# facebookresearch/unbiased-teacher-v2

Hardware: AMD Instinct MI355X
Metric: images/sec/node (labeled+unlabeled) UTv2 step, R50-FPN 1333x800 (higher is better)
Workload: dtype f16

## Files before the change

include/utv2.h:

```cpp
#ifndef UTV2_H
#define UTV2_H
#include <stdint.h>
#ifdef __cplusplus
extern "C" {
#endif

typedef struct ihipStream_t* utv2_stream_t;

int utv2_conv2d_nhwc_fwd(const float* x, const float* w, float* y, const float* scale, const float* bias,
                         const float* residual, int N, int H, int W, int C, int K, int KH, int KW, int stride, int pad,
                         int in_dil, int OH, int OW, int relu, int accumulate, int Kred, utv2_stream_t stream);
int utv2_conv2d_stem_fwd(const float* x, const float* w, void* y, int y_dtype, const float* scale, const float* bias, int N,
                         int H, int W, int K, int KH, int KW, int stride, int pad, int OH, int OW, int relu, int Kred,
                         utv2_stream_t stream);
int utv2_conv2d_wgrad_splits(int N, int OH, int OW, int K, int Kred);
int64_t utv2_conv2d_wgrad_workspace_floats(int N, int OH, int OW, int K, int Kred);
int utv2_conv2d_nhwc_wgrad(const float* x, const float* dy, float* dw, float* ws, int N, int H, int W, int C, int K,
                           int KH, int KW, int stride, int pad, int OH, int OW, int accumulate, utv2_stream_t stream);
int utv2_colsum(const float* g, float* db, float* ws, int M, int C, int accumulate, utv2_stream_t stream);
int utv2_weight_flip_transpose(const float* w, float* wt, int K, int KH, int KW, int C, utv2_stream_t stream);

int utv2_conv2d_ml_fwd(const float* x, const float* w, float* y, const float* scale, const float* bias,
                       const float* residual, int nlev, const int* H_host, const int* W_host, int N, int C, int K, int KH,
                       int KW, int pad, int relu, int accumulate, utv2_stream_t stream);
// ... 230 lines not shown
int utv2_roi_sample(const float* boxes, const unsigned char* valid, const float* max_iou, const int* argmax, const float* keys, int N, int P,
                    const float* gt_boxes, const int* gt_classes, const unsigned char* gt_valid, const float* gt_scores, const float* gt_std,
                    int G, float iou_thr, int num_classes, int batch, int nfg_max, float* out_boxes, int64_t* out_classes,
                    float* out_gt_boxes, unsigned char* out_valid, int64_t* out_idx, float* out_conf, float* out_std, utv2_stream_t stream);
int utv2_roi_box_loss(const float* deltas, const float* stdl, int64_t ld, const int64_t* cls, const float* prop, const float* gtb,
                      const float* gstd, int R, int num_classes, int nbox, int mode, float wx, float wy, float scale_clamp, float ts_better,
                      float t_cert, float* sum, float* gdeltas, float* gstd_out, utv2_stream_t stream);
int utv2_softmax_focal_fwd(const float* logits, const int* target, int R, int C, float gamma, float* loss_sum, float* ws,
                           utv2_stream_t stream);
int utv2_softmax_focal_bwd(const float* logits, const int* target, int R, int C, float gamma, const float* coef,
                           float* dlogits, utv2_stream_t stream);
int utv2_rcnn_loss_combine(const float* rpn_sup, const float* rpn_uns, const float* focal_sup, const float* focal_uns, const float* box_sup,
                           const float* box_uns, const int* tgt_sup, int n_sup, const int* tgt_uns, int n_uns, float rpn_norm_sup,
                           float rpn_norm_uns, float w_rpn_cls, float w_rpn_loc, float w_box, const float* wt_host, float* rec, float* coef,
                           utv2_stream_t stream);

int utv2_stem_pool_fwd_bf16(const void* xpad16, const void* w16s, void* y, const float* scale, const float* shift, int N, int H, int W,
                            int K, utv2_stream_t stream);

int utv2_bottleneck_supported(int C, int MID, int has_shortcut);
int utv2_bottleneck_fwd_bf16(const void* x, void* y, const void* w1, const void* w2, const void* w3, const void* wsc, const float* s1,
                             const float* b1, const float* s2, const float* b2, const float* s3, const float* b3, const float* ssc,
                             const float* bsc, int N, int H, int W, int C, int MID, utv2_stream_t stream);

int64_t utv2_aug_resize_workspace_bytes(int H, int W, int OH, int OW);
int utv2_aug_resize_bilinear_u8(const unsigned char* src, int H, int W, unsigned char* dst, int OH, int OW, int flip, void* ws,
                                utv2_stream_t stream);
int utv2_aug_gray_mean_u8(const unsigned char* img, int64_t npix, void* sum_ws, int* mean_out, utv2_stream_t stream);
int utv2_aug_blend_u8(unsigned char* img, int64_t npix, int mode, float alpha, const int* mean, utv2_stream_t stream);
int utv2_aug_hue_u8(unsigned char* img, int64_t npix, int shift, utv2_stream_t stream);
int utv2_aug_grayscale_u8(unsigned char* img, int64_t npix, utv2_stream_t stream);
int utv2_aug_box_blur_u8(const unsigned char* src, unsigned char* dst, int H, int W, int vertical, int radius, int ww, int fw,
                         utv2_stream_t stream);
int utv2_aug_erase_u8(unsigned char* img, int H, int W, int i, int j, int h, int w, const float* noise, utv2_stream_t stream);
int utv2_aug_hwc_to_chw_u8(const unsigned char* src, unsigned char* dst, int64_t npix, utv2_stream_t stream);

int utv2_coco_pair_keys(const float* scores, const int* cls, const long long* off, int N, int K, long long* keys, utv2_stream_t stream);
int utv2_coco_seg_offsets(const long long* keys, int64_t n, int64_t nseg, long long* off, utv2_stream_t stream);
int utv2_coco_rank_keys(const long long* key1, const long long* pair_off, int64_t D, int K, int max_dets, long long* key2,
                        unsigned char* rank, utv2_stream_t stream);
int64_t utv2_coco_eval_workspace_bytes(int64_t D, int K);
int utv2_coco_match(const float* dbox, const long long* dperm, const long long* dpair_off, const double* gbox, const unsigned char* gcrowd,
                    const double* garea, const long long* gperm, const long long* gpair_off, int N, int K, int64_t D, int max_dets,
                    int max_gt, const double* iou_thrs_host, const double* area_rng_host, void* ws, utv2_stream_t stream);
int utv2_coco_accumulate(const long long* perm2, const long long* cat_off, const unsigned char* rank, int K, int64_t D,
                         const double* rec_thrs_host, const void* ws, double* precision, double* recall, utv2_stream_t stream);
// ... 16 lines not shown
```

unbiased-teacher-v2_amd/csrc/bottleneck.hip:

```cpp
#include "common.h"

#define BT_TH 8
#define BT_TW 16
#define BT_HW 18
#define BT_HALO 180
#define BT_HP 192
#define BT_COUT 256
#define BT_MID 64
#define BT_STAGE 16384
#define BT_C1 (BT_HP * 128)
#define BT_PRM 1280
#define BT_LDS (BT_STAGE + BT_C1 + BT_PRM * 4)

struct BtArgs {
  const h16_t* x;
  h16_t* y;
  const h16_t *w1, *w2, *w3, *wsc;
  const float *s1, *b1, *s2, *b2, *s3, *b3, *ssc, *bsc;
  int N, H, W, tiles_x, tiles_y, ntiles;
};

__device__ __forceinline__ bf16x8_t lds_frag(const unsigned char* smem, int off) { return *(const bf16x8_t*)(smem + off); }

template <int CIN, bool SC>
__global__ __launch_bounds__(256, 3) void bottleneck_fused(BtArgs a) {
  constexpr int NCH = CIN / 32;
  extern __shared__ __attribute__((aligned(16))) unsigned char smem[];
  unsigned char* stageA = smem;
  unsigned char* c1 = smem + BT_STAGE;
  unsigned char* stageB = smem + BT_STAGE;
  unsigned char* c2 = smem;
  unsigned char* w3l = smem + BT_STAGE;
  float* prm = (float*)(smem + BT_STAGE + BT_C1);
  const int tid = threadIdx.x, lane = tid & 63, wave = tid >> 6, l31 = lane & 31, fh = lane >> 5;

  int t;
  {
    const int bid = blockIdx.x, q = a.ntiles >> 3, r = a.ntiles & 7, xcd = bid & 7, idx = bid >> 3;
    t = (xcd < r ? xcd * (q + 1) : r * (q + 1) + (xcd - r) * q) + idx;
  }
  const int per = a.tiles_x * a.tiles_y;
  const int n = t / per, rem = t - n * per, ty = rem / a.tiles_x, tx = rem - ty * a.tiles_x;
  const int y0 = ty * BT_TH, x0 = tx * BT_TW;
  const h16_t* ximg = a.x + (size_t)n * a.H * a.W * CIN;

  const h16_t* xsrc[3];
  int xdst[3];
#pragma unroll
// ... 73 lines not shown
      *(bf16x8_t*)(nxt + wdst) = wr[(kc + 1) % 3];
    }
    __syncthreads();
  }

  {
    const int pbs[3] = {pbA, pbA, pbB}, cbs[3] = {0, 1, cbB};
#pragma unroll
    for (int i = 0; i < 3; ++i) {
      const int px = pbs[i] * 32 + l31;
      const int hy = px / BT_HW, hx = px - hy * BT_HW, gy = y0 - 1 + hy, gx = x0 - 1 + hx;
      const bool ok = px < BT_HALO && gy >= 0 && gy < a.H && gx >= 0 && gx < a.W;
#pragma unroll
      for (int q = 0; q < 4; ++q) {
        const int ch = cbs[i] * 32 + 8 * q + 4 * fh;
        const f32x4 sc = *(const f32x4*)(prm + ch), bi = *(const f32x4*)(prm + 64 + ch);
        bf16x4_t o;
#pragma unroll
        for (int j = 0; j < 4; ++j) {
          float v = acc1[i][4 * q + j] * sc[j] + bi[j];
          v = ok ? fmaxf(v, 0.f) : 0.f;
          o[j] = (h16_t)v;
        }
        *(bf16x4_t*)(c1 + px * 128 + (((cbs[i] * 4 + q) ^ (px & 7)) << 4) + fh * 8) = o;
      }
    }
  }
#pragma unroll
  for (int i = 0; i < 2; ++i) *(bf16x8_t*)(stageA + t2co[i] * 128 + ((t2slot ^ (t2co[i] & 7)) << 4)) = tr[0][i];
  __syncthreads();

  f32x16 acc2[2];
#pragma unroll
  for (int i = 0; i < 2; ++i)
#pragma unroll
    for (int e = 0; e < 16; ++e) acc2[i][e] = 0.f;
  const int p = wave * 32 + l31, pr = p >> 4, pc = p & 15;
  const int qco[2] = {tid >> 3, (tid + 256) >> 3}, qslot = tid & 7;
  bf16x8_t wq[2], sq[2];
#pragma unroll
  for (int tap = 0; tap < 9; ++tap) {
    unsigned char* cur = stageA + (tap & 1) * 8192;
    unsigned char* nxt = stageA + ((tap + 1) & 1) * 8192;
    if (tap + 3 < 9) {
#pragma unroll
      for (int i = 0; i < 2; ++i) tr[tap % 3][i] = *(const bf16x8_t*)(a.w2 + t2co[i] * 576 + (tap + 3) * 64 + t2slot * 8);
    } else if (tap == 6) {
#pragma unroll
      for (int i = 0; i < 2; ++i) {
        wq[i] = *(const bf16x8_t*)(a.w3 + qco[i] * BT_MID + qslot * 8);
        if constexpr (SC) sq[i] = *(const bf16x8_t*)(a.wsc + qco[i] * CIN + qslot * 8);
      }
    }
    const int dy = tap / 3, dx = tap - dy * 3;
    const int h = (pr + dy) * BT_HW + pc + dx;
#pragma unroll
    for (int ks = 0; ks < 4; ++ks) {
      const int slot = ks * 2 + fh;
      const bf16x8_t xf = lds_frag(c1, h * 128 + ((slot ^ (h & 7)) << 4));
      const bf16x8_t wa = lds_frag(cur, w0row * 128 + ((slot ^ (w0row & 7)) << 4));
      const bf16x8_t wb = lds_frag(cur, w1row * 128 + ((slot ^ (w1row & 7)) << 4));
      acc2[0] = mfma_32x32x16(wa, xf, acc2[0]);
      acc2[1] = mfma_32x32x16(wb, xf, acc2[1]);
    }
    if (tap + 1 < 9) {
#pragma unroll
      for (int i = 0; i < 2; ++i) *(bf16x8_t*)(nxt + t2co[i] * 128 + ((t2slot ^ (t2co[i] & 7)) << 4)) = tr[(tap + 1) % 3][i];
    }
    __syncthreads();
  }
  const int sub = lane >> 3, cv = lane & 7;
  int opix[4];
#pragma unroll
  for (int i = 0; i < 4; ++i) {
    const int pp = wave * 32 + 8 * i + sub, gy = y0 + (pp >> 4), gx = x0 + (pp & 15);
    opix[i] = (gy < a.H && gx < a.W) ? ((gy * a.W + gx) * BT_COUT + cv * 8) : -1;
  }
  h16_t* yout = a.y + (size_t)n * a.H * a.W * BT_COUT;
  bf16x8_t res[2][4];
  bf16x8_t xf3[4];
  if constexpr (!SC) {
#pragma unroll
    for (int i = 0; i < 4; ++i) res[0][i] = opix[i] >= 0 ? *(const bf16x8_t*)(ximg + opix[i]) : zero8;
  } else {
    const int gy = y0 + pr, gx = x0 + pc;
    const bool in = gy < a.H && gx < a.W;
#pragma unroll
    for (int ks = 0; ks < 4; ++ks)
      xf3[ks] = in ? *(const bf16x8_t*)(ximg + ((size_t)gy * a.W + gx) * CIN + ks * 16 + fh * 8) : zero8;
  }
#pragma unroll
  for (int cb = 0; cb < 2; ++cb)
#pragma unroll
    for (int q = 0; q < 4; ++q) {
// ... 133 lines not shown
}

extern "C" {

int utv2_bottleneck_fwd_bf16(const void* x, void* y, const void* w1, const void* w2, const void* w3, const void* wsc, const float* s1,
                             const float* b1, const float* s2, const float* b2, const float* s3, const float* b3, const float* ssc,
                             const float* bsc, int N, int H, int W, int C, int MID, hipStream_t stream) {
  if (!x || !y || x == y || !w1 || !w2 || !w3 || !s1 || !b1 || !s2 || !b2 || !s3 || !b3 || N < 1 || H < 1 || W < 1) return UTV2_EARG;
  if (MID != BT_MID || !((C == 256 && !wsc) || (C == 64 && wsc && ssc && bsc))) return UTV2_EARG;
  if ((long long)H * W * BT_COUT > 0x7fffffffll) return UTV2_EARG;
  BtArgs a;
  a.x = (const h16_t*)x; a.y = (h16_t*)y; a.w1 = (const h16_t*)w1; a.w2 = (const h16_t*)w2; a.w3 = (const h16_t*)w3; a.wsc = (const h16_t*)wsc;
  a.s1 = s1; a.b1 = b1; a.s2 = s2; a.b2 = b2; a.s3 = s3; a.b3 = b3; a.ssc = ssc; a.bsc = bsc;
  a.N = N; a.H = H; a.W = W;
  a.tiles_x = cdiv(W, BT_TW); a.tiles_y = cdiv(H, BT_TH);
  const long long nt = (long long)N * a.tiles_x * a.tiles_y;
  if (nt > 0x7fffffff) return UTV2_EARG;
  a.ntiles = (int)nt;
  if (wsc) hipLaunchKernelGGL((bottleneck_fused<64, true>), dim3((unsigned)a.ntiles), dim3(256), BT_LDS, stream, a);
  else hipLaunchKernelGGL((bottleneck_fused<256, false>), dim3((unsigned)a.ntiles), dim3(256), BT_LDS, stream, a);
  return utv2_launch_status();
}

int utv2_bottleneck_supported(int C, int MID, int has_shortcut) {
  return MID == BT_MID && ((C == 256 && !has_shortcut) || (C == 64 && has_shortcut));
}

}
```

unbiased-teacher-v2_amd/ubteacher/hip.py:

```python
import ctypes
import os

import torch

_HERE = os.path.dirname(os.path.abspath(__file__))
_LIB_DIR = os.environ.get("UTV2_LIB_DIR") or os.path.join(os.path.dirname(_HERE), "lib")
LIB_PATH = os.path.join(_LIB_DIR, "libutv2_hip.so")
LIB_PATHS = {"bf16": LIB_PATH, "fp16": os.path.join(_LIB_DIR, "libutv2_hip_f16.so")}
H16 = ["bf16"]


_H16_DT = [torch.bfloat16]


def set_h16(kind):
    assert kind in LIB_PATHS
    H16[0] = kind
    _H16_DT[0] = torch.bfloat16 if kind == "bf16" else torch.float16


def h16_dtype():
    return _H16_DT[0]

_lib = None
# ... 989 lines not shown
        ri = rowinfo_nhwc(N, H, W, OH, OW, stride, pad, kh, kw, x.device)
    if relu_bits is not None:
        assert out.dtype == h16_dtype()
        relu_bits = _bits_ok(relu_bits, out.shape)
    call("utv2_conv2d_nhwc_fwd_bf16_bits", _p(x), _dt(x), _p(w16), _p(out), _same_dt(out, residual, mask, post_mask), _p(scale), _p(bias),
         _p(residual), _p(mask), _p(post_mask), N, H, W, C, K, kh, kw, stride, pad, in_dil, OH, OW, int(relu), int(accumulate), _p(ri),
         _p(relu_bits), None, None, _stream())
    return out


def bottleneck_fwd_bf16(x, w1, w2, w3, s1, b1, s2, b2, s3, b3, wsc=None, ssc=None, bsc=None, out=None):
    N, H, W, C = x.shape
    MID, K = w1.shape[0], w3.shape[0]
    assert x.dtype == h16_dtype() and w1.dtype == w2.dtype == w3.dtype == h16_dtype() and K == 256
    assert tuple(w1.shape) == (MID, C) and tuple(w2.shape) == (MID, 9 * MID) and tuple(w3.shape) == (K, MID)
    assert wsc is None or (tuple(wsc.shape) == (K, C) and wsc.dtype == h16_dtype())
    if out is None:
        out = torch.empty((N, H, W, K), dtype=x.dtype, device=x.device)
    call("utv2_bottleneck_fwd_bf16", _p(x), _p(out), _p(w1), _p(w2), _p(w3), _p(wsc), _p(s1), _p(b1), _p(s2), _p(b2), _p(s3), _p(b3),
         _p(ssc), _p(bsc), N, H, W, C, MID, _stream())
    return out


def bottleneck_supported(C, MID, has_shortcut):
    return bool(load().utv2_bottleneck_supported(C, MID, int(has_shortcut)))


def conv2d_dgrad_bf16(dy, wt16, in_shape, stride, pad, kh, kw, out=None, out_dtype=None, mask=None, residual=None, post_mask=None,
                      mask_bits=None, post_mask_bits=None):
    N, H, W, C = in_shape
    _, OH, OW, K = dy.shape
    if out is None:
        out = torch.empty((N, H, W, C), dtype=_act_dtype(dy, out_dtype), device=dy.device)
    ri = None
    if _CONV_ROWINFO and kh * kw > 1 and stride == 1 and dy.dtype == h16_dtype() and K % 32 == 0 and kh * kw <= 16 and OW < 32768:
        ri = rowinfo_nhwc(N, OH, OW, H, W, 1, kh - 1 - pad, kh, kw, dy.device)
    if mask_bits is not None or post_mask_bits is not None:
        assert out.dtype == h16_dtype() and (mask is None or mask_bits is None) and (post_mask is None or post_mask_bits is None)
        mask_bits = _bits_ok(mask_bits, out.shape) if mask_bits is not None else None
        post_mask_bits = _bits_ok(post_mask_bits, out.shape) if post_mask_bits is not None else None
    call("utv2_conv2d_nhwc_fwd_bf16_bits", _p(dy), _dt(dy), _p(wt16), _p(out), _same_dt(out, residual, mask, post_mask), None, None,
         _p(residual), _p(mask), _p(post_mask), N, OH, OW, K, C, kh, kw, 1, kh - 1 - pad, stride, H, W, 0, 0, _p(ri), None,
         _p(mask_bits), _p(post_mask_bits), _stream())
    return out


# ... 398 lines not shown
```

unbiased-teacher-v2_amd/ubteacher/modeling/backbone.py:

```python
import math
import os

import torch

from .. import hip, ops
from ..d2.registry import BACKBONE_REGISTRY


def _nchw_view(cout, cin, k):
    def fn(t):
        return t.view(cout, k, k, cin).permute(0, 3, 1, 2)
    return fn


def _msra_init(cout, cin, k):
    def fn(t):
        std = math.sqrt(2.0 / (cout * k * k))
        t.normal_(0.0, std)
    return fn


def _xavier_init(cout, cin, k):
    def fn(t):
        bound = math.sqrt(3.0 / (cin * k * k))
# ... 101 lines not shown
                 stride_in_1x1=True):
        self.out_features = out_features
        def stem_init(t):
            t.zero_()
            w = torch.empty(64, 7, 7, 3, device=t.device).normal_(0.0, math.sqrt(2.0 / (64 * 49)))
            t.view(64, 208)[:, :196].view(64, 7, 7, 4)[..., :3].copy_(w)
        stem_train = freeze_at < 1
        self.stem_w = store.new((64, 208), "decay" if stem_train else "frozen", stem_init).export(
            prefix + ".stem.conv1.weight", lambda t: torch.as_strided(t, (64, 3, 7, 7), (208, 1, 28, 4), t.storage_offset()))
        self.stem_bn = folder.add(FrozenBN(store, prefix + ".stem.conv1.norm", 64))
        self.stem = ops.Conv(self.stem_w, 4, 64, 7, 2, 3, bn=self.stem_bn, relu=True, trainable=stem_train, kred=208)
        self.stages = []
        cin = 64
        for si, nblocks in enumerate(num_blocks):
            name, mid, cout = "res%d" % (si + 2), groups * width_per_group * 2 ** si, 256 * 2 ** si
            trainable = freeze_at < si + 2
            blocks = []
            for b in range(nblocks):
                stride = 2 if (b == 0 and name != "res2") else 1
                blocks.append(Bottleneck(store, folder, "%s.%s.%d" % (prefix, name, b), cin, cout, mid, stride, trainable, groups,
                                         stride_in_1x1))
                cin = cout
            self.stages.append((name, blocks, trainable))
        self.channels = {"res2": 256, "res3": 512, "res4": 1024, "res5": 2048}
        self.strides = {"res2": 4, "res3": 8, "res4": 16, "res5": 32}

    def __call__(self, x4):
        outs = {}
        if self.stem.trainable and torch.is_grad_enabled():
            assert x4.dtype == torch.float32 and x4.shape[-1] == 4, "a trainable stem takes the fp32 NHWC4 image"
            x = ops.stem(self.stem, x4)
            for name, blocks, trainable in self.stages:
                for b in blocks:
                    x = b(x)
                if name in self.out_features:
                    outs[name] = x
            return outs
        sc, sh = self.stem.scale_shift()
        if x4.dtype == hip.h16_dtype():
            v = (self.stem_w.store.version, hip.H16[0])
            if getattr(self, "_w16s_version", None) != v:
                self._w16s = hip.stem_weight_image(self.stem_w.t)
                self._w16s_version = v
            if os.environ.get("UTV2_FUSED_STEM_POOL", "1") != "0" and self._w16s.shape[0] == 64:
                x = hip.stem_pool_fwd_bf16(x4, self._w16s, sc, sh)
            else:
                x = hip.maxpool3x3s2(hip.conv2d_stem_fwd_bf16(x4, self._w16s, sc, sh, True, hip.h16_dtype()))
        else:
            x = hip.maxpool3x3s2(hip.conv2d_stem_fwd(x4, self.stem_w.t, sc, sh, 2, 3, 7, 7, True, ops.act_dtype()))
        for name, blocks, trainable in self.stages:
            if trainable:
                for b in blocks:
                    x = b(x)
            else:
                with torch.no_grad():
                    for b in blocks:
                        x = b(x)
            if name in self.out_features:
                outs[name] = x
        return outs


def ResNet50(store, folder, prefix, out_features, freeze_at=2):
    return ResNet(store, folder, prefix, out_features, freeze_at)


def build_resnet(cfg, store, folder, prefix):
    blocks, groups, wpg, s1x1 = resnet_spec(cfg)
    return ResNet(store, folder, prefix, cfg.MODEL.RESNETS.OUT_FEATURES, cfg.MODEL.BACKBONE.FREEZE_AT, blocks, groups, wpg, s1x1)


def _conv_bias(store, prefix, cin, cout, k, stride, pad, init, relu=False):
    w = store.new((cout, k * k * cin), "decay", init(cout, cin, k)).export(prefix + ".weight", _nchw_view(cout, cin, k))
    b = store.new((cout,), "decay", lambda t: t.zero_()).export(prefix + ".bias")
    return ops.Conv(w, cin, cout, k, stride, pad, bias=b, relu=relu, trainable=True)


class FPN:

    def __init__(self, store, folder, cfg, top_block_kind):
# ... 85 lines not shown
```

unbiased-teacher-v2_amd/ubteacher/ops.py:

```python
import os

import torch

from . import hip

_HOOKS = {}
PRECISION = ["fp32"]


def set_precision(p):
    assert p in ("fp32", "bf16", "fp16")
    PRECISION[0] = p
    hip.set_h16("fp16" if p == "fp16" else "bf16")


def amp():
    return PRECISION[0] != "fp32"


def act_dtype():
    return hip.h16_dtype() if amp() else torch.float32


_VERSION = [0]
# ... 320 lines not shown

    def dgrad_cout(self):
        if self.k == 3 and self.stride == 1 and self.cout % 32 and self.cout % 8 == 0 and (self.cout > 32 or self.dgrad_pad_small):
            return (self.cout + 31) // 32 * 32
        return self.cout

    def use_bf16(self):
        return amp() and self.cin % 8 == 0 and self.kred == self.k * self.k * self.cin

    def use_bf16_wgrad(self):
        return (amp() and self.cin % 8 == 0 and self.cout % 8 == 0 and self.k * self.k <= 16
                and self.kred == self.k * self.k * self.cin)

    def gn_stats_fused(self):
        return self.gn_cpg == 8 and self.cout % 8 == 0 and not self.relu and os.environ.get("UTV2_GN_STATS_FUSED", "1") != "0"

    def bias_grad_from_gn(self):
        return self.bias_by_gn and self.bias is not None and self.trainable and self.use_bf16_wgrad() and self.use_bf16_dgrad() \
            and os.environ.get("UTV2_GN_BIAS_GRAD", "1") != "0"

    def use_bf16_dgrad(self):
        return amp() and self.cout % 8 == 0

    def __call__(self, x, residual=None, out=None, colscale_handle=None, meta=None):
        if torch.is_grad_enabled() and self.trainable:
            return _ConvFn.apply(x, residual, hook(x.device), self, (out, getattr(x, "_utv2_fanin", None), getattr(x, "_utv2_pair", None)),
                                 colscale_handle, meta)
        return self._forward(x, residual, out, colscale_handle, meta)

    def gconv_weight(self):
        return self.w.store.bf16(self.w) if amp() else self.w.t

    def _forward(self, x, residual, out, cs, meta, relu_bits=None):
        sc, sh = self.scale_shift()
        if self.gconv:
            assert meta is None and residual is None and out is None and cs is None and relu_bits is None
            w = self.gconv_weight()
            if x.dtype != w.dtype:
                raise RuntimeError("grouped conv: %s activation with %s weights (layer cout=%d)" % (x.dtype, w.dtype, self.cout))
            return hip.gconv3x3_fwd(x.contiguous(), w, self.groups, self.stride, sc, sh, self.relu,
                                    out_dtype=torch.float32 if self.out_fp32 else x.dtype)
        b16 = self.use_bf16()
        w = self.w.store.bf16(self.w) if b16 else self.w.t
        kw = {}
        if b16:
            kw["out_dtype"] = out.dtype if out is not None else (torch.float32 if self.out_fp32 else hip.h16_dtype())
        else:
            assert x.dtype == torch.float32, "the fp32 conv kernels take fp32 activations (layer cin=%d)" % self.cin
        if not b16 and not x.is_contiguous():
            x = x.contiguous()
        if self.groups > 1:
            assert meta is not None and self.k > 1 and residual is None and out is None and cs is None
        if meta is not None and self.k > 1:
            assert self.stride == 1 and self.pad == (self.k - 1) // 2
            if b16:
                part = None
                if self.gn_stats_fused() and out is None and residual is None and kw["out_dtype"] == hip.h16_dtype() and self.cin % 32 == 0:
                    part = hip.gn_part_buffer(x.shape[0], self.cout, x.device)
                y = hip.conv2d_ml_fwd_bf16(x, w, meta.level_hw, meta.N, scale=sc, bias=sh, residual=residual, k=self.k, pad=self.pad,
                                           relu=self.relu, out=out, groups=self.groups, gn_part=part, **kw)
                self._gn_part = (y.data_ptr(), part) if part is not None else None
            elif self.groups > 1:
                Kg = self.cout // self.groups
                y = torch.cat([hip.conv2d_ml_fwd(x[:, gi * self.cin:(gi + 1) * self.cin].contiguous(), w[gi * Kg:(gi + 1) * Kg], meta.level_hw,
                                                 meta.N, scale=None, bias=None if sh is None else sh[gi * Kg:(gi + 1) * Kg], k=self.k,
                                                 pad=self.pad, relu=self.relu) for gi in range(self.groups)], dim=1)
            else:
                y = hip.conv2d_ml_fwd(x, w, meta.level_hw, meta.N, scale=sc, bias=sh, residual=residual, k=self.k, pad=self.pad,
                                      relu=self.relu, out=out, **kw)
        elif meta is not None:
            fn = hip.conv2d_fwd_bf16 if b16 else hip.conv2d_fwd
            y = fn(x.view(1, x.shape[0], 1, x.shape[1]), w, scale=sc, bias=sh,
                   residual=None if residual is None else residual.view(1, x.shape[0], 1, -1), relu=self.relu,
                   out=None if out is None else out.view(1, x.shape[0], 1, -1), **kw).view(x.shape[0], self.cout)
        else:
            fn = hip.conv2d_fwd_bf16 if b16 else hip.conv2d_fwd
            if relu_bits is not None:
                kw["relu_bits"] = relu_bits
            y = fn(x, w, scale=sc, bias=sh, residual=residual, stride=self.stride, pad=self.pad, relu=self.relu, kh=self.k,
                   kw=self.k, out=out, **kw)
        if cs is not None:
            assert y.dtype == torch.float32
            if meta is not None and _scale_ml_on() and y.is_contiguous():
                hip.scale_cols_ml(y, meta.rows, self.colscale, [h.t for h in cs])
            elif meta is not None:
                for l, h in enumerate(cs):
                    r0, r1 = meta.rows[l]
                    hip.scale_cols(y[r0:r1], self.colscale, h.t)
            else:
                hip.scale_cols(y.view(-1, self.cout), self.colscale, cs.t)
        return y


class _ConvFn(torch.autograd.Function):
    @staticmethod
    def forward(ctx, x, residual, hk, layer, out_holder, cs, meta):
        out = out_holder[0]
        y = layer._forward(x, residual, out, cs, meta)
        ctx.layer = layer
        ctx.cs = cs
        ctx.meta = meta
        ctx.has_res = residual is not None
        ctx.x_bits = _bits_of(x) if (layer.premask_input and meta is None) else None
# ... 148 lines not shown

    @staticmethod
    def _backward_grouped(ctx, dy):
        layer = ctx.layer
        x, y = ctx.saved_tensors
        w = layer.gconv_weight()
        g = dy.contiguous()
        if g.dtype != w.dtype:
            g = g.to(w.dtype)
        relu = layer.relu and not (layer.grad_premasked and premask_on())
        if relu:
            g = hip.relu_bwd_scale(g, y if y.dtype == g.dtype else y.to(g.dtype), None)
        sc, _ = layer.scale_shift()
        dx = None
        if ctx.needs_input_grad[0]:
            pm = x if (layer.premask_input and premask_on()) else None
            dx = hip.gconv3x3_dgrad(g, w, layer.groups, layer.stride, tuple(x.shape), scale=sc, mask=pm, out_dtype=x.dtype)
        _wgrad_launch(lambda: hip.gconv3x3_wgrad(x, g, layer.w.g, layer.groups, layer.stride, scale=sc, accumulate=True), x, g, key=layer)
        if GRAD_SYNC[0] is not None:
            GRAD_SYNC[0].on_backward_done(_sync_handles(layer))
        return dx, None, None, None, None, None, None


def _wgrad16(layer, x4, g4):
    if layer.gconv:
        _wgrad_launch(lambda: hip.gconv3x3_wgrad(x4, g4, layer.w.g, layer.groups, layer.stride, scale=layer.bn.scale, accumulate=True),
                      x4, g4, key=layer)
        return
    n_, h_, w_, _ = x4.shape
    ri = hip.rowinfo_nhwc(n_, h_, w_, g4.shape[1], g4.shape[2], layer.stride, layer.pad, layer.k, layer.k, x4.device)
    _wgrad_launch(lambda: hip.conv2d_wgrad_bf16(x4, g4.reshape(-1, layer.cout), layer.w.g, ri, layer.cin, layer.k, layer.k, accumulate=True,
                                                rowscale=layer.bn.scale), x4, g4, key=layer)


def _dgrad16(layer, g4, in_shape, mask=None, residual=None, post_mask=None, mask_bits=None, post_mask_bits=None):
    if mask_bits is not None:
        mask = None
    if post_mask_bits is not None:
        post_mask = None
    if layer.gconv:
        assert post_mask is None and post_mask_bits is None and mask_bits is None
        return hip.gconv3x3_dgrad(g4, layer.gconv_weight(), layer.groups, layer.stride, tuple(in_shape), scale=layer.bn.scale, mask=mask,
                                  residual=residual, out_dtype=hip.h16_dtype())
    BITS_STATS["reads"] += (mask_bits is not None) + (post_mask_bits is not None)
    return hip.conv2d_dgrad_bf16(g4, layer.wt16(layer.bn.scale), tuple(in_shape), layer.stride, layer.pad, layer.k, layer.k,
                                 out_dtype=hip.h16_dtype(), mask=mask, residual=residual, post_mask=post_mask, mask_bits=mask_bits,
                                 post_mask_bits=post_mask_bits)


class GradHandoff:
    _live = []

    def __init__(self):
# ... 19 lines not shown
    return premask_on() and os.environ.get("UTV2_GRAD_HANDOFF", "1") != "0"


def relu_bits_on():
    return os.environ.get("UTV2_RELU_BITS", "1") != "0"


BITS_STATS = {"planes": 0, "reads": 0}


def _bits_of(t):
    b = getattr(t, "_utv2_relu_bits", None)
    if b is not None and (b[0] != t.data_ptr() or b[1] != t._version):
        return None
    return None if b is None else b[2]


def premask_on():
    return os.environ.get("UTV2_PREMASK", "1") != "0"


class _BottleneckFn(torch.autograd.Function):
    @staticmethod
    def forward(ctx, x, hk, block):
        c1, c2, c3, cs = block.conv1, block.conv2, block.conv3, block.shortcut
        res = cs._forward(x, None, None, None, None) if cs is not None else x
        b1 = b2 = b3 = None
        if relu_bits_on() and all(c.relu and c.cout % 8 == 0 for c in (c1, c2, c3)):
            planes, (n_, h_, w_, _) = [], x.shape
            for c in (c1, c2, c3):
                h_, w_ = hip.conv_out_size(h_, c.k, c.stride, c.pad), hip.conv_out_size(w_, c.k, c.stride, c.pad)
                planes.append(hip.relu_bits_buffer((n_, h_, w_, c.cout), x.device))
            if c2.gconv:
                planes[0] = planes[1] = None
            b1, b2, b3 = planes
            BITS_STATS["planes"] += sum(b is not None for b in planes)
        y1 = c1._forward(x, None, None, None, None, relu_bits=b1)
        y2 = c2._forward(y1, None, None, None, None, relu_bits=b2)
        y3 = c3._forward(y2, res, None, None, None, relu_bits=b3)
        ctx.block = block
        ctx.handoff = None
        if ctx.needs_input_grad[0] and grad_handoff_on() and getattr(x, "_utv2_handoff", None) is None:
            ctx.handoff = x._utv2_handoff = GradHandoff()
        ctx.bits = (_bits_of(x), b1, b2)
        if b3 is not None:
            y3._utv2_relu_bits = (y3.data_ptr(), y3._version, b3)
        ctx.save_for_backward(x, y1, y2, y3)
        if GRAD_SYNC[0] is not None:
            for l in (c1, c2, c3, cs):
                if l is not None:
                    GRAD_SYNC[0].on_forward(_sync_handles(l))
        return y3

    @staticmethod
    def backward(ctx, dy):
        block = ctx.block
        c1, c2, c3, cs = block.conv1, block.conv2, block.conv3, block.shortcut
        x, y1, y2, y3 = ctx.saved_tensors
        pre = premask_on()
        if pre and block.grad_premasked:
            gm = dy.contiguous()
        else:
            gm = hip.relu_bwd_scale(dy.contiguous(), y3, None)
        pm = x if (pre and block.input_relu) else None
        bx, b1, b2 = ctx.bits
        if pm is None:
            bx = None
        _wgrad16(c3, y2, gm)
        g2 = _dgrad16(c3, gm, y2.shape, mask=y2, mask_bits=b2)
        _wgrad16(c2, y1, g2)
        g1 = _dgrad16(c2, g2, y1.shape, mask=y1, mask_bits=b1)
        _wgrad16(c1, x, g1)
        if cs is not None:
            _wgrad16(cs, x, gm)
        dx = None
        if ctx.needs_input_grad[0]:
            parked = ctx.handoff.take() if ctx.handoff is not None else None
            if parked is not None and (parked.dtype != hip.h16_dtype() or tuple(parked.shape) != tuple(x.shape)):
                raise RuntimeError("GradHandoff: parked gradient of another shape / type")
            if cs is None:
                dx = _dgrad16(c1, g1, x.shape, residual=gm, post_mask=pm, post_mask_bits=bx)
                if parked is not None:
                    dx = dx + parked
            elif c1.stride == 2:
                c = hip.conv2d_fwd_bf16(gm, cs.wt16(cs.bn.scale), out_dtype=hip.h16_dtype())
                c = hip.conv2d_fwd_bf16(g1, c1.wt16(c1.bn.scale), residual=c, out_dtype=hip.h16_dtype())
                dx = hip.zero_interleave2x(c, x.shape[1], x.shape[2], mask=pm if bx is None else None, mask_bits=bx if pm is not None else None,
                                           add=parked)
                BITS_STATS["reads"] += (bx is not None and pm is not None)
            elif cs.stride == 2:
                assert c1.stride == 1 and cs.k == 1 and cs.pad == 0
                c = hip.conv2d_fwd_bf16(gm, cs.wt16(cs.bn.scale), out_dtype=hip.h16_dtype())
                d = hip.zero_interleave2x(c, x.shape[1], x.shape[2], add=parked)
                dx = _dgrad16(c1, g1, x.shape, residual=d, post_mask=pm, post_mask_bits=bx)
            else:
                d = _dgrad16(cs, gm, x.shape, residual=parked)
                dx = _dgrad16(c1, g1, x.shape, residual=d, post_mask=pm, post_mask_bits=bx)
        if GRAD_SYNC[0] is not None:
            for l in (c3, c2, c1, cs):
                if l is not None:
                    GRAD_SYNC[0].on_backward_done(_sync_handles(l))
        return dx, None, None


def _fused_frozen_block_on():
    return os.environ.get("UTV2_FUSED_FROZEN_BLOCK", "1") != "0"


def bottleneck(block, x):
    convs = [c for c in (block.conv1, block.conv2, block.conv3, block.shortcut) if c is not None]
    fused = (amp() and torch.is_grad_enabled() and x.dtype == hip.h16_dtype()
             and all(c.trainable and c.bn is not None and c.bias is None
                     and (c.gconv or (c.use_bf16() and c.use_bf16_wgrad() and c.use_bf16_dgrad())) for c in convs)
             and block.conv1.stride in (1, 2) and block.conv1.k == 1 and block.conv3.k == 1
             and not (block.conv1.gconv or block.conv3.gconv)
             and (block.conv1.stride == 1 or block.conv2.stride == 1)
             and (block.shortcut is None or block.shortcut.stride == max(block.conv1.stride, block.conv2.stride)))
    if fused:
        return _BottleneckFn.apply(x, hook(x.device), block)
    if (amp() and x.dtype == hip.h16_dtype() and x.is_contiguous() and _fused_frozen_block_on()
            and (not torch.is_grad_enabled() or not any(c.trainable for c in convs)) and not x.requires_grad
            and all(c.stride == 1 for c in convs) and block.conv1.k == 1 and block.conv2.k == 3 and block.conv3.k == 1
            and (block.shortcut is None or block.shortcut.k == 1) and block.conv3.cout == 256
            and all(c.bn is not None and c.bias is None and c.use_bf16() for c in convs)
            and x.shape[1] * x.shape[2] * 256 < 2 ** 31
            and block.conv2.groups == 1 and block.conv1.cout <= 64
            and hip.bottleneck_supported(block.conv1.cin, block.conv1.cout, block.shortcut is not None)):
        st = block.conv1.w.store
        (s1, b1), (s2, b2), (s3, b3) = block.conv1.scale_shift(), block.conv2.scale_shift(), block.conv3.scale_shift()
        kw = {}
        if block.shortcut is not None:
            ssc, bsc = block.shortcut.scale_shift()
            kw = dict(wsc=st.bf16(block.shortcut.w), ssc=ssc, bsc=bsc)
        return hip.bottleneck_fwd_bf16(x, st.bf16(block.conv1.w), st.bf16(block.conv2.w), st.bf16(block.conv3.w), s1, b1, s2, b2, s3, b3, **kw)
    sc = block.shortcut(x) if block.shortcut is not None else x
    out = block.conv1(x)
    out = block.conv2(out)
    return block.conv3(out, residual=sc)


class _StemFn(torch.autograd.Function):

    @staticmethod
    def forward(ctx, x4, hk, layer):
        sc, sh = layer.scale_shift()
        y = hip.conv2d_stem_fwd(x4, layer.w.t, sc, sh, layer.stride, layer.pad, layer.k, layer.k, True, act_dtype())
        ctx.layer = layer
        ctx.save_for_backward(x4, y)
        if GRAD_SYNC[0] is not None:
            GRAD_SYNC[0].on_forward(_sync_handles(layer))
# ... 487 lines not shown
```

Baseline: 345.0.

## Emit stride-2 subsampled output from last frozen res2 bottleneck for res3 1x1 stride-2 convs

Adds a variant of the fused frozen bottleneck kernel that computes conv2/conv3 only at even-position pixels and writes a quarter-size output. The first res3 block, whose conv1 and shortcut are 1x1 stride 2, then runs them at stride 1 on this compact input, including in wgrad. The aim is to skip three quarters of the conv2/conv3 work and the full-resolution res2 output write and read when res2 is not an output feature. In exchange it adds a new kernel path, a per-call stride override plumbed through the conv and autograd code, and tight config checks. Only half the waves do conv2 MFMA work in the new path.

Result: no change. 348.1, median of 6 (+0.9%).

```diff
diff --git a/include/utv2.h b/include/utv2.h
--- a/include/utv2.h
+++ b/include/utv2.h
@@ -276,6 +276,9 @@
 int utv2_bottleneck_fwd_bf16(const void* x, void* y, const void* w1, const void* w2, const void* w3, const void* wsc, const float* s1,
                              const float* b1, const float* s2, const float* b2, const float* s3, const float* b3, const float* ssc,
                              const float* bsc, int N, int H, int W, int C, int MID, utv2_stream_t stream);
+int utv2_bottleneck_fwd_bf16_s2out(const void* x, void* y, const void* w1, const void* w2, const void* w3, const float* s1, const float* b1,
+                                   const float* s2, const float* b2, const float* s3, const float* b3, int N, int H, int W, int C, int MID,
+                                   utv2_stream_t stream);
 
 int64_t utv2_aug_resize_workspace_bytes(int H, int W, int OH, int OW);
 int utv2_aug_resize_bilinear_u8(const unsigned char* src, int H, int W, unsigned char* dst, int OH, int OW, int flip, void* ws,
diff --git a/unbiased-teacher-v2_amd/csrc/bottleneck.hip b/unbiased-teacher-v2_amd/csrc/bottleneck.hip
--- a/unbiased-teacher-v2_amd/csrc/bottleneck.hip
+++ b/unbiased-teacher-v2_amd/csrc/bottleneck.hip
@@ -22,8 +22,11 @@
 
 __device__ __forceinline__ bf16x8_t lds_frag(const unsigned char* smem, int off) { return *(const bf16x8_t*)(smem + off); }
 
-template <int CIN, bool SC>
+__device__ __forceinline__ int bt_s2_row(int hy, int hx) { return hy * BT_HW + (hx >> 1) + (hx & 1) * 9; }
+
+template <int CIN, bool SC, bool S2 = false>
 __global__ __launch_bounds__(256, 3) void bottleneck_fused(BtArgs a) {
+  static_assert(!(S2 && SC), "the quarter-row form exists for the identity block");
   constexpr int NCH = CIN / 32;
   extern __shared__ __attribute__((aligned(16))) unsigned char smem[];
   unsigned char* stageA = smem;
@@ -143,7 +146,12 @@
           v = ok ? fmaxf(v, 0.f) : 0.f;
           o[j] = (h16_t)v;
         }
-        *(bf16x4_t*)(c1 + px * 128 + (((cbs[i] * 4 + q) ^ (px & 7)) << 4) + fh * 8) = o;
+        if constexpr (S2) {
+          const int hr = px < BT_HALO ? bt_s2_row(hy, hx) : px;
+          *(bf16x4_t*)(c1 + hr * 128 + (((cbs[i] * 4 + q) ^ ((hr >> 1) & 7)) << 4) + fh * 8) = o;
+        } else {
+          *(bf16x4_t*)(c1 + px * 128 + (((cbs[i] * 4 + q) ^ (px & 7)) << 4) + fh * 8) = o;
+        }
       }
     }
   }
@@ -156,7 +164,9 @@
   for (int i = 0; i < 2; ++i)
 #pragma unroll
     for (int e = 0; e < 16; ++e) acc2[i][e] = 0.f;
-  const int p = wave * 32 + l31, pr = p >> 4, pc = p & 15;
+  const int p = S2 ? l31 : wave * 32 + l31, pr = S2 ? (l31 & 3) : (p >> 4), pc = S2 ? (l31 >> 2) : (p & 15);
+  const int wu = __builtin_amdgcn_readfirstlane(wave);
+  bf16x8_t wf3[2][4];
   const int qco[2] = {tid >> 3, (tid + 256) >> 3}, qslot = tid & 7;
   bf16x8_t wq[2], sq[2];
 #pragma unroll
@@ -167,22 +177,43 @@
 #pragma unroll
       for (int i = 0; i < 2; ++i) tr[tap % 3][i] = *(const bf16x8_t*)(a.w2 + t2co[i] * 576 + (tap + 3) * 64 + t2slot * 8);
     } else if (tap == 6) {
-#pragma unroll
-      for (int i = 0; i < 2; ++i) {
-        wq[i] = *(const bf16x8_t*)(a.w3 + qco[i] * BT_MID + qslot * 8);
-        if constexpr (SC) sq[i] = *(const bf16x8_t*)(a.wsc + qco[i] * CIN + qslot * 8);
+      if constexpr (S2) {
+#pragma unroll
+        for (int u = 0; u < 2; ++u)
+#pragma unroll
+          for (int ks = 0; ks < 4; ++ks)
+            wf3[u][ks] = *(const bf16x8_t*)(a.w3 + (wu * 64 + u * 32 + l31) * BT_MID + (ks * 2 + fh) * 8);
+      } else {
+#pragma unroll
+        for (int i = 0; i < 2; ++i) {
+          wq[i] = *(const bf16x8_t*)(a.w3 + qco[i] * BT_MID + qslot * 8);
+          if constexpr (SC) sq[i] = *(const bf16x8_t*)(a.wsc + qco[i] * CIN + qslot * 8);
+        }
       }
     }
     const int dy = tap / 3, dx = tap - dy * 3;
-    const int h = (pr + dy) * BT_HW + pc + dx;
-#pragma unroll
-    for (int ks = 0; ks < 4; ++ks) {
-      const int slot = ks * 2 + fh;
-      const bf16x8_t xf = lds_frag(c1, h * 128 + ((slot ^ (h & 7)) << 4));
-      const bf16x8_t wa = lds_frag(cur, w0row * 128 + ((slot ^ (w0row & 7)) << 4));
-      const bf16x8_t wb = lds_frag(cur, w1row * 128 + ((slot ^ (w1row & 7)) << 4));
-      acc2[0] = mfma_32x32x16(wa, xf, acc2[0]);
-      acc2[1] = mfma_32x32x16(wb, xf, acc2[1]);
+    if constexpr (S2) {
+      if (wu < 2) {
+        const int h = bt_s2_row(2 * pr + dy, 2 * pc + dx), wrow = wu * 32 + l31;
+#pragma unroll
+        for (int ks = 0; ks < 4; ++ks) {
+          const int slot = ks * 2 + fh;
+          const bf16x8_t xf = lds_frag(c1, h * 128 + ((slot ^ ((h >> 1) & 7)) << 4));
+          const bf16x8_t wa = lds_frag(cur, wrow * 128 + ((slot ^ (wrow & 7)) << 4));
+          acc2[0] = mfma_32x32x16(wa, xf, acc2[0]);
+        }
+      }
+    } else {
+      const int h = (pr + dy) * BT_HW + pc + dx;
+#pragma unroll
+      for (int ks = 0; ks < 4; ++ks) {
+        const int slot = ks * 2 + fh;
+        const bf16x8_t xf = lds_frag(c1, h * 128 + ((slot ^ (h & 7)) << 4));
+        const bf16x8_t wa = lds_frag(cur, w0row * 128 + ((slot ^ (w0row & 7)) << 4));
+        const bf16x8_t wb = lds_frag(cur, w1row * 128 + ((slot ^ (w1row & 7)) << 4));
+        acc2[0] = mfma_32x32x16(wa, xf, acc2[0]);
+        acc2[1] = mfma_32x32x16(wb, xf, acc2[1]);
+      }
     }
     if (tap + 1 < 9) {
 #pragma unroll
@@ -191,6 +222,80 @@
     __syncthreads();
   }
   const int sub = lane >> 3, cv = lane & 7;
+  if constexpr (S2) {
+    const int Ho = (a.H + 1) >> 1, Wo = (a.W + 1) >> 1;
+    int xpix[4], ypix[4];
+#pragma unroll
+    for (int i = 0; i < 4; ++i) {
+      const int pp = 8 * i + sub, gy = y0 + 2 * (pp & 3), gx = x0 + 2 * (pp >> 2);
+      const bool in = gy < a.H && gx < a.W;
+      xpix[i] = in ? ((gy * a.W + gx) * BT_COUT + wu * 64 + cv * 8) : -1;
+      ypix[i] = in ? (((gy >> 1) * Wo + (gx >> 1)) * BT_COUT + wu * 64 + cv * 8) : -1;
+    }
+    h16_t* yout = a.y + (size_t)n * Ho * Wo * BT_COUT;
+    bf16x8_t res[4];
+#pragma unroll
+    for (int i = 0; i < 4; ++i) res[i] = xpix[i] >= 0 ? *(const bf16x8_t*)(ximg + xpix[i]) : zero8;
+    if (wu < 2) {
+#pragma unroll
+      for (int q = 0; q < 4; ++q) {
+        const int ch = wu * 32 + 8 * q + 4 * fh;
+        const f32x4 sc = *(const f32x4*)(prm + 128 + ch), bi = *(const f32x4*)(prm + 192 + ch);
+        bf16x4_t o;
+#pragma unroll
+        for (int j = 0; j < 4; ++j) o[j] = (h16_t)fmaxf(acc2[0][4 * q + j] * sc[j] + bi[j], 0.f);
+        *(bf16x4_t*)(c2 + p * 128 + (((wu * 4 + q) ^ (p & 7)) << 4) + fh * 8) = o;
+      }
+    }
+    __syncthreads();
+    bf16x8_t cf[4];
+#pragma unroll
+    for (int ks = 0; ks < 4; ++ks) cf[ks] = lds_frag(c2, p * 128 + (((ks * 2 + fh) ^ (p & 7)) << 4));
+    __syncthreads();
+    float* patch = (float*)smem + wave * (16 * 64);
+    f32x16 acc3[2];
+#pragma unroll
+    for (int u = 0; u < 2; ++u)
+#pragma unroll
+      for (int e = 0; e < 16; ++e) acc3[u][e] = 0.f;
+#pragma unroll
+    for (int ks = 0; ks < 4; ++ks)
+#pragma unroll
+      for (int u = 0; u < 2; ++u) acc3[u] = mfma_32x32x16(wf3[u][ks], cf[ks], acc3[u]);
+    const f32x4 s3a = *(const f32x4*)(prm + 256 + wu * 64 + cv * 8), s3b = *(const f32x4*)(prm + 256 + wu * 64 + cv * 8 + 4);
+    const f32x4 b3a = *(const f32x4*)(prm + 512 + wu * 64 + cv * 8), b3b = *(const f32x4*)(prm + 512 + wu * 64 + cv * 8 + 4);
+#pragma unroll
+    for (int hh = 0; hh < 2; ++hh) {
+      if ((l31 >> 4) == hh) {
+        const int prow = l31 & 15;
+#pragma unroll
+        for (int u = 0; u < 2; ++u)
+#pragma unroll
+          for (int q = 0; q < 4; ++q) {
+            const int cl = u * 32 + 8 * q + 4 * fh;
+            const f32x4 v = {acc3[u][4 * q], acc3[u][4 * q + 1], acc3[u][4 * q + 2], acc3[u][4 * q + 3]};
+            *(f32x4*)(patch + prow * 64 + (((cl >> 2) ^ prow) << 2)) = v;
+          }
+      }
+      __builtin_amdgcn_s_waitcnt(0xc07f);
+      __builtin_amdgcn_wave_barrier();
+#pragma unroll
+      for (int i2 = 0; i2 < 2; ++i2) {
+        const int i = hh * 2 + i2, prow = 8 * i2 + sub;
+        const f32x4 v0 = *(const f32x4*)(patch + prow * 64 + (((2 * cv) ^ prow) << 2)), v1 = *(const f32x4*)(patch + prow * 64 + (((2 * cv + 1) ^ prow) << 2));
+        bf16x8_t o;
+#pragma unroll
+        for (int j = 0; j < 4; ++j) {
+          o[j] = (h16_t)fmaxf(v0[j] * s3a[j] + b3a[j] + (float)res[i][j], 0.f);
+          o[4 + j] = (h16_t)fmaxf(v1[j] * s3b[j] + b3b[j] + (float)res[i][4 + j], 0.f);
+        }
+        if (ypix[i] >= 0) *(bf16x8_t*)(yout + ypix[i]) = o;
+      }
+      __builtin_amdgcn_s_waitcnt(0xc07f);
+      __builtin_amdgcn_wave_barrier();
+    }
+    return;
+  }
   int opix[4];
 #pragma unroll
   for (int i = 0; i < 4; ++i) {
@@ -370,6 +475,24 @@
   return utv2_launch_status();
 }
 
+int utv2_bottleneck_fwd_bf16_s2out(const void* x, void* y, const void* w1, const void* w2, const void* w3, const float* s1, const float* b1,
+                                   const float* s2, const float* b2, const float* s3, const float* b3, int N, int H, int W, int C, int MID,
+                                   hipStream_t stream) {
+  if (!x || !y || x == y || !w1 || !w2 || !w3 || !s1 || !b1 || !s2 || !b2 || !s3 || !b3 || N < 1 || H < 1 || W < 1) return UTV2_EARG;
+  if (MID != BT_MID || C != 256) return UTV2_EARG;
+  if ((long long)H * W * BT_COUT > 0x7fffffffll) return UTV2_EARG;
+  BtArgs a;
+  a.x = (const h16_t*)x; a.y = (h16_t*)y; a.w1 = (const h16_t*)w1; a.w2 = (const h16_t*)w2; a.w3 = (const h16_t*)w3; a.wsc = nullptr;
+  a.s1 = s1; a.b1 = b1; a.s2 = s2; a.b2 = b2; a.s3 = s3; a.b3 = b3; a.ssc = nullptr; a.bsc = nullptr;
+  a.N = N; a.H = H; a.W = W;
+  a.tiles_x = cdiv(W, BT_TW); a.tiles_y = cdiv(H, BT_TH);
+  const long long nt = (long long)N * a.tiles_x * a.tiles_y;
+  if (nt > 0x7fffffff) return UTV2_EARG;
+  a.ntiles = (int)nt;
+  hipLaunchKernelGGL((bottleneck_fused<256, false, true>), dim3((unsigned)a.ntiles), dim3(256), BT_LDS, stream, a);
+  return utv2_launch_status();
+}
+
 int utv2_bottleneck_supported(int C, int MID, int has_shortcut) {
   return MID == BT_MID && ((C == 256 && !has_shortcut) || (C == 64 && has_shortcut));
 }
diff --git a/unbiased-teacher-v2_amd/ubteacher/hip.py b/unbiased-teacher-v2_amd/ubteacher/hip.py
--- a/unbiased-teacher-v2_amd/ubteacher/hip.py
+++ b/unbiased-teacher-v2_amd/ubteacher/hip.py
@@ -1035,6 +1035,19 @@
     return out
 
 
+def bottleneck_fwd_bf16_s2out(x, w1, w2, w3, s1, b1, s2, b2, s3, b3, out=None):
+    N, H, W, C = x.shape
+    MID, K = w1.shape[0], w3.shape[0]
+    assert x.dtype == h16_dtype() and w1.dtype == w2.dtype == w3.dtype == h16_dtype() and K == 256
+    assert tuple(w1.shape) == (MID, C) and tuple(w2.shape) == (MID, 9 * MID) and tuple(w3.shape) == (K, MID)
+    if out is None:
+        out = torch.empty((N, (H + 1) // 2, (W + 1) // 2, K), dtype=x.dtype, device=x.device)
+    assert tuple(out.shape) == (N, (H + 1) // 2, (W + 1) // 2, K) and out.dtype == x.dtype
+    call("utv2_bottleneck_fwd_bf16_s2out", _p(x), _p(out), _p(w1), _p(w2), _p(w3), _p(s1), _p(b1), _p(s2), _p(b2), _p(s3), _p(b3),
+         N, H, W, C, MID, _stream())
+    return out
+
+
 def bottleneck_supported(C, MID, has_shortcut):
     return bool(load().utv2_bottleneck_supported(C, MID, int(has_shortcut)))
 
diff --git a/unbiased-teacher-v2_amd/ubteacher/modeling/backbone.py b/unbiased-teacher-v2_amd/ubteacher/modeling/backbone.py
--- a/unbiased-teacher-v2_amd/ubteacher/modeling/backbone.py
+++ b/unbiased-teacher-v2_amd/ubteacher/modeling/backbone.py
@@ -147,6 +147,11 @@
                                          stride_in_1x1))
                 cin = cout
             self.stages.append((name, blocks, trainable))
+        last2, first3 = self.stages[0][1][-1], self.stages[1][1][0]
+        self.quarter_rows_cfg = ops.quarter_rows_config_ok(
+            "res2" in out_features, freeze_at >= 2, stride_in_1x1,
+            (last2.conv1.cin, last2.conv1.cout, last2.conv3.cout, last2.conv2.groups),
+            tuple((c.k, c.stride) if c is not None else None for c in (first3.conv1, first3.shortcut)))
         self.channels = {"res2": 256, "res3": 512, "res4": 1024, "res5": 2048}
         self.strides = {"res2": 4, "res3": 8, "res4": 16, "res5": 32}
 
@@ -173,14 +178,20 @@
                 x = hip.maxpool3x3s2(hip.conv2d_stem_fwd_bf16(x4, self._w16s, sc, sh, True, hip.h16_dtype()))
         else:
             x = hip.maxpool3x3s2(hip.conv2d_stem_fwd(x4, self.stem_w.t, sc, sh, 2, 3, 7, 7, True, ops.act_dtype()))
+        reader_ok = (self.quarter_rows_cfg and ops.res2_quarter_rows_on()
+                     and ops.quarter_rows_reader_ok(self.stages[1][1][0], x))
+        compact = False
         for name, blocks, trainable in self.stages:
             if trainable:
                 for b in blocks:
-                    x = b(x)
+                    x, compact = ops.bottleneck(b, x, compact_in=compact), False
             else:
                 with torch.no_grad():
                     for b in blocks:
-                        x = b(x)
+                        if name == "res2" and b is blocks[-1] and reader_ok and ops.quarter_rows_writer_ok(b, x):
+                            x, compact = ops.bottleneck(b, x, s2out=True), True
+                        else:
+                            x, compact = ops.bottleneck(b, x, compact_in=compact), False
             if name in self.out_features:
                 outs[name] = x
         return outs
diff --git a/unbiased-teacher-v2_amd/ubteacher/ops.py b/unbiased-teacher-v2_amd/ubteacher/ops.py
--- a/unbiased-teacher-v2_amd/ubteacher/ops.py
+++ b/unbiased-teacher-v2_amd/ubteacher/ops.py
@@ -366,7 +366,11 @@
     def use_bf16_dgrad(self):
         return amp() and self.cout % 8 == 0
 
-    def __call__(self, x, residual=None, out=None, colscale_handle=None, meta=None):
+    def __call__(self, x, residual=None, out=None, colscale_handle=None, meta=None, stride=None):
+        if stride is not None:
+            if torch.is_grad_enabled() and self.trainable:
+                raise RuntimeError("a per-call stride exists outside autograd and inside the fused bottleneck node only")
+            return self._forward(x, residual, out, colscale_handle, meta, stride=stride)
         if torch.is_grad_enabled() and self.trainable:
             return _ConvFn.apply(x, residual, hook(x.device), self, (out, getattr(x, "_utv2_fanin", None), getattr(x, "_utv2_pair", None)),
                                  colscale_handle, meta)
@@ -375,8 +379,9 @@
     def gconv_weight(self):
         return self.w.store.bf16(self.w) if amp() else self.w.t
 
-    def _forward(self, x, residual, out, cs, meta, relu_bits=None):
+    def _forward(self, x, residual, out, cs, meta, relu_bits=None, stride=None):
         sc, sh = self.scale_shift()
+        assert stride is None or (meta is None and not self.gconv)
         if self.gconv:
             assert meta is None and residual is None and out is None and cs is None and relu_bits is None
             w = self.gconv_weight()
@@ -421,8 +426,8 @@
             fn = hip.conv2d_fwd_bf16 if b16 else hip.conv2d_fwd
             if relu_bits is not None:
                 kw["relu_bits"] = relu_bits
-            y = fn(x, w, scale=sc, bias=sh, residual=residual, stride=self.stride, pad=self.pad, relu=self.relu, kh=self.k,
-                   kw=self.k, out=out, **kw)
+            y = fn(x, w, scale=sc, bias=sh, residual=residual, stride=self.stride if stride is None else stride, pad=self.pad,
+                   relu=self.relu, kh=self.k, kw=self.k, out=out, **kw)
         if cs is not None:
             assert y.dtype == torch.float32
             if meta is not None and _scale_ml_on() and y.is_contiguous():
@@ -617,13 +622,15 @@
         return dx, None, None, None, None, None, None
 
 
-def _wgrad16(layer, x4, g4):
+def _wgrad16(layer, x4, g4, stride=None):
     if layer.gconv:
+        assert stride is None
         _wgrad_launch(lambda: hip.gconv3x3_wgrad(x4, g4, layer.w.g, layer.groups, layer.stride, scale=layer.bn.scale, accumulate=True),
                       x4, g4, key=layer)
         return
     n_, h_, w_, _ = x4.shape
-    ri = hip.rowinfo_nhwc(n_, h_, w_, g4.shape[1], g4.shape[2], layer.stride, layer.pad, layer.k, layer.k, x4.device)
+    ri = hip.rowinfo_nhwc(n_, h_, w_, g4.shape[1], g4.shape[2], layer.stride if stride is None else stride, layer.pad, layer.k, layer.k,
+                          x4.device)
     _wgrad_launch(lambda: hip.conv2d_wgrad_bf16(x4, g4.reshape(-1, layer.cout), layer.w.g, ri, layer.cin, layer.k, layer.k, accumulate=True,
                                                 rowscale=layer.bn.scale), x4, g4, key=layer)
 
@@ -689,20 +696,25 @@
 
 class _BottleneckFn(torch.autograd.Function):
     @staticmethod
-    def forward(ctx, x, hk, block):
+    def forward(ctx, x, hk, block, compact_in=False):
         c1, c2, c3, cs = block.conv1, block.conv2, block.conv3, block.shortcut
-        res = cs._forward(x, None, None, None, None) if cs is not None else x
+        s_in = 1 if compact_in else None
+        if compact_in and (ctx.needs_input_grad[0] or cs is None or c1.stride != 2 or cs.stride != 2 or c1.k != 1 or cs.k != 1):
+            raise RuntimeError("a compact input needs a block whose input convs are 1x1 stride 2 and an input without gradient")
+        ctx.s_in = s_in
+        res = cs._forward(x, None, None, None, None, stride=s_in) if cs is not None else x
         b1 = b2 = b3 = None
         if relu_bits_on() and all(c.relu and c.cout % 8 == 0 for c in (c1, c2, c3)):
             planes, (n_, h_, w_, _) = [], x.shape
             for c in (c1, c2, c3):
-                h_, w_ = hip.conv_out_size(h_, c.k, c.stride, c.pad), hip.conv_out_size(w_, c.k, c.stride, c.pad)
+                st = 1 if (compact_in and c is c1) else c.stride
+                h_, w_ = hip.conv_out_size(h_, c.k, st, c.pad), hip.conv_out_size(w_, c.k, st, c.pad)
                 planes.append(hip.relu_bits_buffer((n_, h_, w_, c.cout), x.device))
             if c2.gconv:
                 planes[0] = planes[1] = None
             b1, b2, b3 = planes
             BITS_STATS["planes"] += sum(b is not None for b in planes)
-        y1 = c1._forward(x, None, None, None, None, relu_bits=b1)
+        y1 = c1._forward(x, None, None, None, None, relu_bits=b1, stride=s_in)
         y2 = c2._forward(y1, None, None, None, None, relu_bits=b2)
         y3 = c3._forward(y2, res, None, None, None, relu_bits=b3)
         ctx.block = block
@@ -737,9 +749,9 @@
         g2 = _dgrad16(c3, gm, y2.shape, mask=y2, mask_bits=b2)
         _wgrad16(c2, y1, g2)
         g1 = _dgrad16(c2, g2, y1.shape, mask=y1, mask_bits=b1)
-        _wgrad16(c1, x, g1)
+        _wgrad16(c1, x, g1, stride=ctx.s_in)
         if cs is not None:
-            _wgrad16(cs, x, gm)
+            _wgrad16(cs, x, gm, stride=ctx.s_in)
         dx = None
         if ctx.needs_input_grad[0]:
             parked = ctx.handoff.take() if ctx.handoff is not None else None
@@ -767,32 +779,73 @@
             for l in (c3, c2, c1, cs):
                 if l is not None:
                     GRAD_SYNC[0].on_backward_done(_sync_handles(l))
-        return dx, None, None
+        return (dx, None, None, None) if ctx.s_in is not None else (dx, None, None)
 
 
 def _fused_frozen_block_on():
     return os.environ.get("UTV2_FUSED_FROZEN_BLOCK", "1") != "0"
 
 
-def bottleneck(block, x):
+def res2_quarter_rows_on():
+    return os.environ.get("UTV2_RES2_QUARTER_ROWS", "1") != "0"
+
+
+def quarter_rows_config_ok(res2_is_output, res2_frozen, stride_in_1x1, last_block_shape, res3_first_block):
+    return (not res2_is_output and res2_frozen and stride_in_1x1 and tuple(last_block_shape) == (256, 64, 256, 1)
+            and tuple(res3_first_block) == ((1, 2), (1, 2)))
+
+
+def _fused_node_ok(block, x):
     convs = [c for c in (block.conv1, block.conv2, block.conv3, block.shortcut) if c is not None]
-    fused = (amp() and torch.is_grad_enabled() and x.dtype == hip.h16_dtype()
+    return (amp() and torch.is_grad_enabled() and x.dtype == hip.h16_dtype()
              and all(c.trainable and c.bn is not None and c.bias is None
                      and (c.gconv or (c.use_bf16() and c.use_bf16_wgrad() and c.use_bf16_dgrad())) for c in convs)
              and block.conv1.stride in (1, 2) and block.conv1.k == 1 and block.conv3.k == 1
              and not (block.conv1.gconv or block.conv3.gconv)
              and (block.conv1.stride == 1 or block.conv2.stride == 1)
              and (block.shortcut is None or block.shortcut.stride == max(block.conv1.stride, block.conv2.stride)))
-    if fused:
-        return _BottleneckFn.apply(x, hook(x.device), block)
-    if (amp() and x.dtype == hip.h16_dtype() and x.is_contiguous() and _fused_frozen_block_on()
+
+
+def _frozen_block_fused_ok(block, x):
+    convs = [c for c in (block.conv1, block.conv2, block.conv3, block.shortcut) if c is not None]
+    return (amp() and x.dtype == hip.h16_dtype() and x.is_contiguous() and _fused_frozen_block_on()
             and (not torch.is_grad_enabled() or not any(c.trainable for c in convs)) and not x.requires_grad
             and all(c.stride == 1 for c in convs) and block.conv1.k == 1 and block.conv2.k == 3 and block.conv3.k == 1
             and (block.shortcut is None or block.shortcut.k == 1) and block.conv3.cout == 256
             and all(c.bn is not None and c.bias is None and c.use_bf16() for c in convs)
             and x.shape[1] * x.shape[2] * 256 < 2 ** 31
             and block.conv2.groups == 1 and block.conv1.cout <= 64
-            and hip.bottleneck_supported(block.conv1.cin, block.conv1.cout, block.shortcut is not None)):
+            and hip.bottleneck_supported(block.conv1.cin, block.conv1.cout, block.shortcut is not None))
+
+
+def quarter_rows_writer_ok(last_block, x):
+    return last_block.shortcut is None and _frozen_block_fused_ok(last_block, x)
+
+
+def quarter_rows_reader_ok(next_block, x):
+    if next_block.shortcut is None or next_block.conv1.gconv or next_block.shortcut.gconv:
+        return False
+    if torch.is_grad_enabled() and any(c.trainable for c in (next_block.conv1, next_block.conv2, next_block.conv3, next_block.shortcut)):
+        return _fused_node_ok(next_block, x)
+    return amp() and x.dtype == hip.h16_dtype() and next_block.conv1.use_bf16() and next_block.shortcut.use_bf16()
+
+
+def bottleneck(block, x, s2out=False, compact_in=False):
+    if s2out:
+        if block.shortcut is not None or not _frozen_block_fused_ok(block, x):
+            raise RuntimeError("the quarter-row form exists for a frozen identity block on the fused kernel only")
+        st = block.conv1.w.store
+        (s1, b1), (s2, b2), (s3, b3) = block.conv1.scale_shift(), block.conv2.scale_shift(), block.conv3.scale_shift()
+        return hip.bottleneck_fwd_bf16_s2out(x, st.bf16(block.conv1.w), st.bf16(block.conv2.w), st.bf16(block.conv3.w), s1, b1, s2, b2, s3, b3)
+    if _fused_node_ok(block, x):
+        return _BottleneckFn.apply(x, hook(x.device), block, True) if compact_in else _BottleneckFn.apply(x, hook(x.device), block)
+    if compact_in:
+        if torch.is_grad_enabled() and any(c.trainable for c in (block.conv1, block.conv2, block.conv3, block.shortcut)):
+            raise RuntimeError("a compact input under autograd needs the fused bottleneck node")
+        sc = block.shortcut(x, stride=1)
+        out = block.conv2(block.conv1(x, stride=1))
+        return block.conv3(out, residual=sc)
+    if _frozen_block_fused_ok(block, x):
         st = block.conv1.w.store
         (s1, b1), (s2, b2), (s3, b3) = block.conv1.scale_shift(), block.conv2.scale_shift(), block.conv3.scale_shift()
         kw = {}
```
